# AnjieCheng/SpatialRGPT

Measured on AMD Instinct MI355X. Metric: region-grounded output tokens/sec @ VILA1.5-8B, 8 regions, greedy, higher is better.
Workload: dtype bf16; 1 GPU; BASELINE configs[1]: SpatialRGPT-VILA1.5-8B geometry (Llama-3-8B 32L/4096/GQA-8 + SigLIP-so400m 384px x2 passes + regiongpt extractor + mlp_downsample), 8 region masks, bs=1 per GPU, prompt 64 ids -> T=259, greedy 128 new tokens; parallelism=dp1, decode=hipGraph, llm_weights=bf16

## Files before the change

### spatialrgpt_amd/csrc/gemv.hip

```cpp
#include <stdlib.h>

#include <type_traits>

#include "common.h"
#include "gemv_route.h"
#include "internal.h"

namespace {

template <typename T>
struct WChunk;
template <>
struct WChunk<bf16_t> {
  static constexpr int VEC = 8;
  static __device__ __forceinline__ void cvt(const u32x4& r, float* f) {
#pragma unroll
    for (int i = 0; i < 4; ++i) {
      f[2 * i] = bf16lo(r[i]);
      f[2 * i + 1] = bf16hi(r[i]);
    }
  }
};
template <>
struct WChunk<float> {
  static constexpr int VEC = 4;
  static __device__ __forceinline__ void cvt(const u32x4& r, float* f) {
#pragma unroll
    for (int i = 0; i < 4; ++i) f[i] = __uint_as_float(r[i]);
  }
};

template <typename T, int B, bool SWIGLU, int NXMAX, int UB = 8>
__global__ __launch_bounds__(256, 2) void gemv_kernel(const T* __restrict__ x, const T* __restrict__ W,
                                                      const T* __restrict__ norm_w, float norm_eps,
                                                      const T* __restrict__ residual, void* __restrict__ out, int N,
                                                      int K, int out_f32) {
  constexpr int VEC = WChunk<T>::VEC;
  constexpr int R = SWIGLU ? 2 : 1;
  constexpr int U = UB / R;
  extern __shared__ __attribute__((aligned(16))) unsigned char smem[];
  T* xs = reinterpret_cast<T*>(smem);
  __shared__ float red[16];
  constexpr int RES_MAXU = 4;
  __shared__ float res_s[B][4][RES_MAXU];

  const int tid = threadIdx.x, lane = tid & 63, wave = tid >> 6;
  const int nchunks = K / VEC;
  const int nit = (nchunks + 63) >> 6;

  u32x4 w[R][U];
  auto issue = [&](int unit, int it0) {
#pragma unroll
    for (int r = 0; r < R; ++r) {
      const u32x4* p = reinterpret_cast<const u32x4*>(W + (size_t)(unit + r * N) * K);
#pragma unroll
      for (int j = 0; j < U; ++j) {
        w[r][j] = __builtin_nontemporal_load(p + min((it0 + j) * 64 + lane, nchunks - 1));
        __builtin_amdgcn_sched_barrier(0);
      }
    }
  };

  {
    const int total = B * nchunks;
    const bool do_norm = norm_w != nullptr;
    Vec16<T> xr[NXMAX], gr[NXMAX];
    const int rb = tid / (4 * RES_MAXU), rw = (tid / RES_MAXU) & 3, rk = tid % RES_MAXU;
    const int runit = (int)blockIdx.x * 4 + rw + rk * (int)gridDim.x * 4;
    const bool rok = !SWIGLU && residual != nullptr && tid < B * 4 * RES_MAXU && runit < N;
    const T res_raw = (residual != nullptr ? residual : x)[rok ? (size_t)rb * N + runit : 0];
#pragma unroll
    for (int j = 0; j < NXMAX; ++j) {
      const int c = (tid + 256 * j) % total;
      xr[j] = *reinterpret_cast<const Vec16<T>*>(x + (size_t)c * VEC);
      gr[j] = *reinterpret_cast<const Vec16<T>*>((do_norm ? norm_w : x) + (size_t)(c % nchunks) * VEC);
    }
    __builtin_amdgcn_sched_barrier(0);
    issue(min((int)blockIdx.x * 4 + wave, N - 1), 0);
    __builtin_amdgcn_sched_barrier(0);
    float ss[B];
#pragma unroll
    for (int b = 0; b < B; ++b) ss[b] = 0.f;
#pragma unroll
    for (int j = 0; j < NXMAX; ++j) {
      const int c = tid + 256 * j;
      const bool ok = c < total;
      float sq = 0.f;
#pragma unroll
      for (int i = 0; i < VEC; ++i) sq += xr[j].get(i) * xr[j].get(i);
      const int b = (B == 1) ? 0 : (c % total) / nchunks;
#pragma unroll
      for (int bb = 0; bb < B; ++bb) ss[bb] += (ok && bb == b) ? sq : 0.f;
    }
    for (int c = tid + 256 * NXMAX; c < total; c += 256) {
      const Vec16<T> v = *reinterpret_cast<const Vec16<T>*>(x + (size_t)c * VEC);
      *reinterpret_cast<Vec16<T>*>(xs + (size_t)c * VEC) = v;
      const int b = c / nchunks;
      float sq = 0.f;
#pragma unroll
      for (int i = 0; i < VEC; ++i) sq += v.get(i) * v.get(i);
#pragma unroll
      for (int bb = 0; bb < B; ++bb)
        if (bb == b) ss[bb] += sq;
    }
    if (rok) res_s[rb][rw][rk] = to_f(res_raw);
    float rs[B];
#pragma unroll
    for (int b = 0; b < B; ++b) rs[b] = 1.f;
    if (do_norm) {
#pragma unroll
      for (int b = 0; b < B; ++b) rs[b] = rsqrtf(block_sum(ss[b], red) / (float)K + norm_eps);
    }
#pragma unroll
    for (int j = 0; j < NXMAX; ++j) {
      const int c = tid + 256 * j;
      if (c < total) {
        Vec16<T> v = xr[j];
        if (do_norm) {
          const int b = (B == 1) ? 0 : c / nchunks;
          float r = rs[0];
#pragma unroll
          for (int bb = 1; bb < B; ++bb)
            if (bb == b) r = rs[bb];
#pragma unroll
          for (int i = 0; i < VEC; ++i) v.set(i, gr[j].get(i) * rnd<T>(xr[j].get(i) * r));
        }
        *reinterpret_cast<Vec16<T>*>(xs + (size_t)c * VEC) = v;
      }
    }
    if (do_norm) {
      for (int c = tid + 256 * NXMAX; c < total; c += 256) {
        const int b = c / nchunks, kc = c - b * nchunks;
        Vec16<T> v = *reinterpret_cast<Vec16<T>*>(xs + (size_t)c * VEC);
        const Vec16<T> g = *reinterpret_cast<const Vec16<T>*>(norm_w + (size_t)kc * VEC);
        float r = rs[0];
#pragma unroll
        for (int bb = 1; bb < B; ++bb)
          if (bb == b) r = rs[bb];
#pragma unroll
        for (int i = 0; i < VEC; ++i) v.set(i, g.get(i) * rnd<T>(v.get(i) * r));
        *reinterpret_cast<Vec16<T>*>(xs + (size_t)c * VEC) = v;
      }
    }
    __syncthreads();
  }

  int uk = 0;
  for (int unit = blockIdx.x * 4 + wave; unit < N; unit += gridDim.x * 4, ++uk) {
    float acc[R][B];
#pragma unroll
    for (int r = 0; r < R; ++r)
#pragma unroll
      for (int b = 0; b < B; ++b) acc[r][b] = 0.f;

    for (int it0 = 0; it0 < nit; it0 += U) {
#pragma unroll
      for (int j = 0; j < U; ++j) {
        const int ch = (it0 + j) * 64 + lane;
        const bool valid = ch < nchunks;
        const int chc = valid ? ch : nchunks - 1;
        float wf[R][VEC];
#pragma unroll
        for (int r = 0; r < R; ++r) {
          u32x4 wv = w[r][j];
#pragma unroll
          for (int q = 0; q < 4; ++q) wv[q] = valid ? wv[q] : 0u;
          WChunk<T>::cvt(wv, wf[r]);
        }
#pragma unroll
        for (int b = 0; b < B; ++b) {
          const Vec16<T> xv = *reinterpret_cast<const Vec16<T>*>(xs + (size_t)b * K + (size_t)chc * VEC);
#pragma unroll
          for (int i = 0; i < VEC; ++i) {
            const float xf = xv.get(i);
#pragma unroll
            for (int r = 0; r < R; ++r) acc[r][b] = fmaf(wf[r][i], xf, acc[r][b]);
          }
        }
      }
      {
        const bool more = it0 + U < nit;
        issue(more ? unit : min(unit + (int)gridDim.x * 4, N - 1), more ? it0 + U : 0);
      }
    }

#pragma unroll
    for (int b = 0; b < B; ++b) {
      float a[R];
#pragma unroll
      for (int r = 0; r < R; ++r) a[r] = wave_sum(acc[r][b]);
      if (lane == 0) {
        if (SWIGLU) {
          const float g = rnd<T>(a[0]), u = rnd<T>(a[R - 1]);
          reinterpret_cast<T*>(out)[(size_t)b * N + unit] = from_f<T>(rnd<T>(silu(g)) * u);
        } else {
          float v = rnd<T>(a[0]);
          if (residual) v = rnd<T>((uk < RES_MAXU ? res_s[b][wave][uk] : to_f(residual[(size_t)b * N + unit])) + v);
          if (out_f32)
            reinterpret_cast<float*>(out)[(size_t)b * N + unit] = v;
          else
            reinterpret_cast<T*>(out)[(size_t)b * N + unit] = from_f<T>(v);
        }
      }
    }
  }
}

template <bool SWIGLU, bool NORM, int NIT, int UB = 8>
__global__ __launch_bounds__(256, 2) void gemv_reg_kernel(const bf16_t* __restrict__ x, const bf16_t* __restrict__ W,
                                                          const bf16_t* __restrict__ norm_w, float norm_eps,
                                                          const bf16_t* __restrict__ residual, void* __restrict__ out, int N,
                                                          int K, int out_f32) {
  typedef bf16_t T;
  constexpr int VEC = 8;
  constexpr int R = SWIGLU ? 2 : 1;
  constexpr int U = UB / R;
  constexpr int RES_MAXU = 4;
  const int tid = threadIdx.x, lane = tid & 63, wave = tid >> 6;
  const int nchunks = K / VEC;

  u32x4 w[R][U];
  auto issue = [&](int unit, auto it0_c) {
    constexpr int IT0 = decltype(it0_c)::value;
#pragma unroll
    for (int r = 0; r < R; ++r) {
      const u32x4* p = reinterpret_cast<const u32x4*>(W + (size_t)(unit + r * N) * K);
#pragma unroll
      for (int j = 0; j < U; ++j) {
        if (IT0 + j < NIT) {
          w[r][j] = __builtin_nontemporal_load(p + min((IT0 + j) * 64 + lane, nchunks - 1));
          __builtin_amdgcn_sched_barrier(0);
        }
      }
    }
  };

  u32x4 xp[NIT];
  unsigned int res_raw;
// ... 65 lines not shown
        }
      }
    };
    batch(std::integral_constant<int, 0>{});
    if constexpr (U < NIT) batch(std::integral_constant<int, U>{});
    if constexpr (2 * U < NIT) batch(std::integral_constant<int, 2 * U>{});
    if constexpr (3 * U < NIT) batch(std::integral_constant<int, 3 * U>{});
    static_assert(4 * U >= NIT, "gemv_reg_kernel: at most 4 batches per row");
    float a[R];
#pragma unroll
    for (int r = 0; r < R; ++r) a[r] = wave_sum(acc[r]);
    const float res_b = __uint_as_float((unsigned int)__builtin_amdgcn_readlane((int)res_raw, uk < RES_MAXU ? uk : 0) << 16);
    if (lane == 0) {
      if (SWIGLU) {
        const float g = rnd<T>(a[0]), u = rnd<T>(a[R - 1]);
        reinterpret_cast<T*>(out)[unit] = from_f<T>(rnd<T>(silu(g)) * u);
      } else {
        float v = rnd<T>(a[0]);
        if (residual) v = rnd<T>((uk < RES_MAXU ? res_b : to_f(residual[unit])) + v);
        if (out_f32)
          reinterpret_cast<float*>(out)[unit] = v;
        else
          reinterpret_cast<T*>(out)[unit] = from_f<T>(v);
      }
    }
  }
}

template <typename T>
int launch_gemv(GemvFamily family, const DecodeProduct& p, hipStream_t s) {
  const GemvValuLaunch l = gemv_valu_launch(family, p.batch, p.N, p.K, sizeof(T) == 2, p.swiglu != 0, srgpt_device_cus());
  SRGPT_CHECK(l.lds <= GEMV_LDS_CAP, SRGPT_ERR_UNSUPPORTED, "srgpt_gemv: batch*K too large for LDS (%zu bytes)", (size_t)l.lds);
  const T *x = (const T*)p.x, *W = (const T*)p.W, *norm_w = (const T*)p.norm_w, *residual = (const T*)p.residual;
  SRGPT_TRY((srgpt_switch<false, true>(p.swiglu != 0, "SWIGLU", [&](auto sw_c) {
    constexpr bool SW = decltype(sw_c)::value;
    if constexpr (sizeof(T) == 2) {
      if (family == GEMV_REG)
        return srgpt_switch<5, 8, 14>(l.NIT, "NIT", [&](auto nit_c) {
          hipLaunchKernelGGL((gemv_reg_kernel<SW, false, decltype(nit_c)::value>), dim3(l.grid), dim3(256), 0, s, x, W, norm_w, p.eps,
                             residual, p.out, p.N, p.K, p.out_f32);
          return (int)SRGPT_OK;
        });
    }
    return srgpt_switch<1, 2, 3, 4>(l.B, "B", [&](auto b_c) {
      return srgpt_switch<2, 8>(l.NX, "NX", [&](auto nx_c) {
        constexpr int B = decltype(b_c)::value, NX = decltype(nx_c)::value;
        const auto go = [&](auto ub_c) {
          constexpr auto kfn = &gemv_kernel<T, B, SW, NX, decltype(ub_c)::value>;
          return srgpt_launch_dyn_lds<kfn>(l.raise_lds_limit ? GEMV_LDS_CAP : 0, dim3(l.grid), dim3(256), (size_t)l.lds, s, x, W, norm_w,
                                           p.eps, residual, p.out, p.N, p.K, p.out_f32);
        };
        if constexpr (!SW && NX == 8) {
          if (l.UB == 7) return go(std::integral_constant<int, 7>{});
        }
        return go(std::integral_constant<int, 8>{});
      });
    });
  })));
  SRGPT_LAUNCH_CHECK();
  return SRGPT_OK;
}

}

int srgpt_decode_product(const DecodeProduct& p, hipStream_t s) {
  const bool bf16 = p.dtype == SRGPT_BF16;
  const GemvRoute r = gemv_route(p.batch, p.K, bf16, p.fp8 != 0, p.norm_w != nullptr);
  const size_t es = dtype_size(p.dtype), on = p.out_f32 ? sizeof(float) : es;
  for (int b0 = 0; b0 < p.batch; b0 += r.chunk) {
    DecodeProduct c = p;
    c.batch = p.batch - b0 < r.chunk ? p.batch - b0 : r.chunk;
    c.x = (const char*)p.x + (size_t)b0 * p.K * es;
    if (p.residual) c.residual = (const char*)p.residual + (size_t)b0 * p.N * es;
    c.out = (char*)p.out + (size_t)b0 * p.N * on;
    if (p.ss_in) c.ss_in = p.ss_in + (size_t)b0 * SRGPT_ROWSS_STRIDE;
    if (p.ss_out) c.ss_out = p.ss_out + (size_t)b0 * SRGPT_ROWSS_STRIDE;
    switch (r.family) {
      case GEMV_SKINNY: SRGPT_TRY(srgpt_skinny_launch(c, s)); break;
      case GEMV_W8: SRGPT_TRY(srgpt_gemv_w8_valu(c, s)); break;
      default: SRGPT_TRY(bf16 ? launch_gemv<bf16_t>(r.family, c, s) : launch_gemv<float>(r.family, c, s));
    }
  }
  return SRGPT_OK;
}

extern "C" int srgpt_gemv(const void* x, const void* W, const void* norm_w, float norm_eps, const void* residual,
                          void* out, int batch, int N, int K, int swiglu, int out_f32, int dtype,
                          srgpt_stream_t stream) {
  SRGPT_CHECK(x && W && out, SRGPT_ERR_ARG, "srgpt_gemv: null pointer");
  SRGPT_CHECK(N > 0 && K > 0 && batch > 0, SRGPT_ERR_ARG, "srgpt_gemv: bad shape");
  SRGPT_CHECK(dtype == SRGPT_F32 || dtype == SRGPT_BF16, SRGPT_ERR_ARG, "srgpt_gemv: bad dtype %d", dtype);
  const int vec = dtype == SRGPT_BF16 ? 8 : 4;
  SRGPT_CHECK(K % vec == 0, SRGPT_ERR_ARG, "srgpt_gemv: K=%d must be a multiple of %d", K, vec);
  SRGPT_CHECK(!(swiglu && (residual || out_f32)), SRGPT_ERR_ARG, "srgpt_gemv: swiglu excludes residual/out_f32");
  return srgpt_decode_product(DecodeProduct{x, W, nullptr, norm_w, norm_eps, residual, out, batch, N, K, swiglu, out_f32, dtype, 0,
                                            nullptr, nullptr, 0},
                              as_stream(stream));
}

static_assert(GEMV_ROWSS_SLOTS == SRGPT_ROWSS_STRIDE, "gemv_route.h counts the slots of include/srgpt.h's tables");
extern "C" int srgpt_gemv_rowss_supported(int batch, int dtype, int fp8) {
// ... 21 lines not shown
```

### spatialrgpt_amd/csrc/internal.h

```cpp
#pragma once
#include "common.h"

struct SrgptGemmEpilogue;
struct GemmRoute;

int srgpt_gemm256_launch(const void* A, const void* W, int K, int lda, const SrgptGemmEpilogue& e, hipStream_t s);
int srgpt_gemm288_launch(const void* A, const void* W, int K, int lda, const SrgptGemmEpilogue& e, hipStream_t s);

void srgpt_splitk_apply(SrgptGemmEpilogue& e, const GemmRoute& r, void* ws);
int srgpt_splitk_finish(const SrgptGemmEpilogue& e, hipStream_t s, bool* fused);

struct DecodeProduct {
  const void *x, *W;
  const float* wscale;
  const void* norm_w;
  float eps;
  const void* residual;
  void* out;
  int batch, N, K, swiglu, out_f32, dtype, fp8;
  const float* ss_in;
  float* ss_out;
  int packed;
};
int srgpt_decode_product(const DecodeProduct& p, hipStream_t s);
int srgpt_skinny_launch(const DecodeProduct& p, hipStream_t s);
int srgpt_gemv_w8_valu(const DecodeProduct& p, hipStream_t s);

int srgpt_decode_attention_pf(const void* qkv, void* kcache, void* vcache, const int* pos, const void* cos_tab,
                              const void* sin_tab, void* out, float* ws, int B, int Hq, int Hkv, int D, int max_pos, int dtype,
                              const void* next_w, int next_n, int next_k, int next_fp8, srgpt_stream_t stream);
void* srgpt_decode_attn_sync_words(float* ws, int B, int Hq, int D, size_t* bytes);

int srgpt_sample_launch(const float* logits, const srgpt_sampling* sp, int64_t* tok, void* ws, float* pv, int* pi, int* err, int B, int V,
                        hipStream_t s);
int srgpt_sample_full_launch(const float* logits, const srgpt_sampling* sp, void* keys_thr, float* pv, int* pi, unsigned* kept_mask, int B,
                             int V, hipStream_t s);

int srgpt_logits_proc_launch(float* scores, const srgpt_logits_proc* lp, const int64_t* ids, int ld, int n, const int* n_dev, int B, int V,
                             hipStream_t s);
int srgpt_logits_proc_max_history();

struct AttnArgs {
  const bf16_t *q, *k, *v;
  bf16_t* o;
  int Tq, Tk, Hq, Hkv, D;
  int64_t q_bs, q_ts, q_hs, k_bs, k_ts, k_hs, v_bs, v_ts, v_hs;
  float scale;
  const int* kv_len;
};
int64_t srgpt_flash_slice_span_limit();
void srgpt_flash_bf16_launch(const AttnArgs& a, int B, bool causal, hipStream_t s);
```

### spatialrgpt_amd/csrc/model.hip

```cpp
#include <vector>

#include "common.h"
#include "gemv_route.h"
#include "internal.h"
#include "pick.h"

namespace {

inline size_t align256(size_t x) { return (x + 255) & ~(size_t)255; }

struct Carver {
  char* base;
  size_t off = 0;
  explicit Carver(void* p) : base(reinterpret_cast<char*>(p)) {}
  void* take(size_t bytes) {
    void* r = base ? base + off : nullptr;
    off += align256(bytes);
    return r;
  }
};

struct VitWs {
  void *col, *h, *qkv, *mlp, *gws;
  size_t gws_bytes, total;
};
VitWs carve_vit(const srgpt_vit_weights* w, int n_img, void* ws) {
  const size_t es = dtype_size(w->dtype);
  const int g = w->image_size / w->patch;
  const size_t rows = (size_t)n_img * (g * g + (w->cls_emb ? 1 : 0));
  Carver c(ws);
  VitWs v;
  v.col = c.take(rows * w->kp * es);
  v.h = c.take(rows * w->hidden * es);
  v.qkv = c.take(rows * 3 * w->hidden * es);
  v.mlp = c.take(rows * w->inter_pad * es);
  v.gws_bytes = (size_t)srgpt_gemm_ws_bytes((int)rows, w->hidden);
  v.gws = c.take(v.gws_bytes);
  v.total = c.off;
  return v;
}

struct LlmWs {
  void *x, *h, *qkv, *attn, *gu, *act, *last;
  void *xd, *qkvd, *attnd, *actd;
  float* dws;
  void* gws;
  size_t gws_bytes;
  float* amax_v;
  int* amax_i;
  int64_t* tok_emb;
  void* smp;
  void* smpf;
  int* err;
  float* rowss;
  void* a8;
  float* a8s;
  size_t total;
};
LlmWs carve_llm(const srgpt_llm_weights* w, int batch, int max_tokens, void* ws) {
  const size_t es = dtype_size(w->dtype);
  const size_t rows = (size_t)batch * max_tokens;
  const size_t qkvw = (size_t)(w->heads + 2 * w->kv_heads) * w->head_dim;
  Carver c(ws);
  LlmWs l;
  l.x = c.take(rows * w->hidden * es);
  l.h = c.take(rows * w->hidden * es);
  l.qkv = c.take(rows * qkvw * es);
  l.attn = c.take(rows * (size_t)w->heads * w->head_dim * es);
  l.gu = c.take(rows * 2 * (size_t)w->inter * es);
  l.act = c.take(rows * (size_t)w->inter * es);
  l.last = c.take((size_t)batch * w->hidden * es);
  l.xd = c.take((size_t)batch * w->hidden * es);
  l.qkvd = c.take((size_t)batch * qkvw * es);
  l.attnd = c.take((size_t)batch * w->heads * w->head_dim * es);
  l.actd = c.take((size_t)batch * w->inter * es);
  l.dws = reinterpret_cast<float*>(c.take((size_t)srgpt_decode_attn_ws_floats(batch, w->heads, w->head_dim) * 4));
  l.gws_bytes = (size_t)srgpt_gemm_ws_bytes((int)rows, (int)(qkvw > (size_t)w->hidden ? qkvw : (size_t)w->hidden));
  l.gws = c.take(l.gws_bytes);
  l.amax_v = reinterpret_cast<float*>(c.take((size_t)batch * PICK_SLICES * 4));
  l.amax_i = reinterpret_cast<int*>(c.take((size_t)batch * PICK_SLICES * 4));
  l.tok_emb = reinterpret_cast<int64_t*>(c.take((size_t)batch * 8));
  l.err = reinterpret_cast<int*>(c.take(sizeof(int)));
  l.smp = c.take((size_t)carve_sample_ws(nullptr, batch).bytes);
  l.smpf = c.take(carve_sample_full_ws(nullptr, batch, w->vocab).head_bytes);
  l.rowss = reinterpret_cast<float*>(c.take((size_t)2 * batch * SRGPT_ROWSS_STRIDE * sizeof(float)));
  l.a8 = nullptr;
  l.a8s = nullptr;
  if (w->fp8_act) {
    size_t kmax = (size_t)w->hidden;
    if ((size_t)w->inter > kmax) kmax = (size_t)w->inter;
    if ((size_t)w->heads * w->head_dim > kmax) kmax = (size_t)w->heads * w->head_dim;
    l.a8 = c.take(rows * kmax);
    l.a8s = reinterpret_cast<float*>(c.take(rows * 4));
  }
  l.total = c.off;
  return l;
}

__global__ void set_int_kernel(int* p, int n, int v) {
  const int i = blockIdx.x * blockDim.x + threadIdx.x;
  if (i < n) p[i] = v;
}

__global__ __launch_bounds__(256) void argmax_partial_kernel(const float* __restrict__ logits, float* __restrict__ pv,
                                                             int* __restrict__ pi, int V) {
  const PickSlice sl = pick_slice(V);
  const float* row = logits + (size_t)blockIdx.y * V;
  float best = -INFINITY;
  int bi = PICK_NONE;
  for (int i = sl.lo + threadIdx.x; i < sl.hi; i += 256) {
    const float v = row[i];
    if (v > best) {
      best = v;
      bi = i;
    }
  }
// ... 72 lines not shown
  const int b = blockIdx.x * blockDim.x + threadIdx.x;
  if (b < B) tok_emb[b] = tok[b];
}

static inline bool advance_embeds(const srgpt_llm_weights* w, const srgpt_llm_state* st) {
  return st->batch <= ADVANCE_MAXB && ((size_t)w->hidden * dtype_size(w->dtype)) % 16 == 0;
}

struct Pick {
  int sampler;
  const srgpt_logits_proc* lp;
};

static int greedy_pick(const srgpt_llm_weights* w, srgpt_llm_state* st, const LlmWs& d, int bump_pos, Pick p, hipStream_t s) {
  const int B = st->batch;
  const bool emb = advance_embeds(w, st);
  if (p.lp) SRGPT_TRY(srgpt_logits_proc_launch(st->logits, p.lp, st->out_ids, st->max_new, 0, st->step, B, w->vocab, s));
  if (st->sampling) {
    if (p.sampler == SRGPT_SAMPLER_FULL)
      SRGPT_TRY(srgpt_sample_full_launch(st->logits, st->sampling, d.smpf, d.amax_v, d.amax_i, nullptr, B, w->vocab, s));
    else
      SRGPT_TRY(srgpt_sample_launch(st->logits, st->sampling, st->tok, d.smp, d.amax_v, d.amax_i, d.err, B, w->vocab, s));
  } else {
    hipLaunchKernelGGL(argmax_partial_kernel, dim3(PICK_SLICES, B), dim3(256), 0, s, st->logits, d.amax_v, d.amax_i, w->vocab);
  }
  hipLaunchKernelGGL(advance_kernel, dim3(1), dim3(B > 4 ? 1024 : 256), 0, s, d.amax_v, d.amax_i, PICK_SLICES, st->tok, st->out_ids,
                     st->pos, st->step, B, st->max_new, bump_pos, emb ? reinterpret_cast<const unsigned char*>(w->embed) : nullptr,
                     reinterpret_cast<unsigned char*>(d.xd), (int)((size_t)w->hidden * dtype_size(w->dtype)), d.tok_emb, st->sampling,
                     p.sampler == SRGPT_SAMPLER_TOPK64 ? 1 : 0);
  SRGPT_LAUNCH_CHECK();
  return SRGPT_OK;
}

}

struct srgpt_graph {
  hipGraph_t graph;
  hipGraphExec_t exec;
};

extern "C" int64_t srgpt_vit_ws_bytes(const srgpt_vit_weights* w, int n_img) {
  if (!w || n_img <= 0) return -1;
  return (int64_t)carve_vit(w, n_img, nullptr).total;
}

extern "C" int srgpt_vit_forward(const srgpt_vit_weights* w, const void* images, void* out, void* ws, int n_img,
                                 srgpt_stream_t stream) {
  SRGPT_CHECK(w && images && out && ws && n_img > 0, SRGPT_ERR_ARG, "srgpt_vit_forward: bad args");
  SRGPT_CHECK(w->hidden % w->heads == 0 && w->image_size >= w->patch, SRGPT_ERR_ARG, "srgpt_vit_forward: bad config");
  SRGPT_CHECK(w->inter_pad >= w->inter && w->inter_pad % 8 == 0, SRGPT_ERR_ARG, "srgpt_vit_forward: inter_pad %d < inter %d",
              w->inter_pad, w->inter);
  const int dt = w->dtype, C = w->hidden, I = w->inter, IP = w->inter_pad, H = w->heads, hd = C / H;
  const int g = w->image_size / w->patch, gg = g * g, L = gg + (w->cls_emb ? 1 : 0), rows = n_img * L;
  const VitWs v = carve_vit(w, n_img, ws);
  void* x = out;
  SRGPT_TRY(srgpt_im2col(images, v.col, n_img, w->image_size, w->patch, w->kp, dt, stream));
  if (!w->cls_emb) {
    SRGPT_TRY(srgpt_gemm(v.col, w->patch_w, w->patch_b, w->pos_emb, x, rows, C, w->kp, w->kp, C, SRGPT_ACT_NONE, 0, L, 0,
                         SRGPT_OUT_PLAIN, 0, v.gws, (int64_t)v.gws_bytes, dt, stream));
  } else {
    SRGPT_TRY(srgpt_gemm(v.col, w->patch_w, w->patch_b, nullptr, v.h, n_img * gg, C, w->kp, w->kp, C, SRGPT_ACT_NONE, 0, 0, 0,
                         SRGPT_OUT_PLAIN, 0, v.gws, (int64_t)v.gws_bytes, dt, stream));
    SRGPT_TRY(srgpt_vit_assemble_cls(v.h, w->cls_emb, w->pos_emb, x, n_img, gg, C, dt, stream));
    if (w->pre_ln_w) SRGPT_TRY(srgpt_layernorm(x, w->pre_ln_w, w->pre_ln_b, x, rows, C, w->eps, SRGPT_ACT_NONE, dt, stream));
  }
  const float scale = 1.0f / sqrtf((float)hd);
  const char* qkv = reinterpret_cast<const char*>(v.qkv);
  const size_t es = dtype_size(dt);
  if (IP > I)
    SRGPT_HIP_TRY(hipMemset2DAsync(reinterpret_cast<char*>(v.mlp) + (size_t)I * es, (size_t)IP * es, 0, (size_t)(IP - I) * es,
                                   (size_t)rows, as_stream(stream)),
// ... 167 lines not shown
    SRGPT_TRY(gemm_w8a8(m.gu, nullptr, l.gu, 2 * I, Hd));
    SRGPT_TRY(srgpt_silu_mul(l.gu, l.act, rows, I, dt, stream));
    SRGPT_TRY(quant(l.act, I));
    return gemm_w8a8(m.down, l.x, l.x, Hd, I);
  }
};

}

static int prefill_impl(const srgpt_llm_weights* w, srgpt_llm_state* st, const void* inputs_embeds, int T, const int* lens,
                        float* all_logits, void* hidden_out, srgpt_stream_t stream) {
  SRGPT_TRY(check_llm(w, st));
  SRGPT_CHECK(inputs_embeds && T > 0 && T <= st->max_pos, SRGPT_ERR_ARG, "srgpt_llm_prefill: T=%d exceeds max_pos=%d", T,
              st->max_pos);
  SRGPT_CHECK(T <= st->ws_tokens, SRGPT_ERR_ARG, "srgpt_llm_prefill: T=%d exceeds ws_tokens=%d", T, st->ws_tokens);
  LlmFormat fmt;
  SRGPT_TRY(llm_format(w, "srgpt_llm_prefill", &fmt));
  const int dt = w->dtype, Hd = w->hidden, I = w->inter, Hq = w->heads, D = w->head_dim;
  const int B = st->batch, rows = B * T;
  if (fmt == FMT_W8A8)
    SRGPT_CHECK(Hd % 128 == 0 && I % 128 == 0 && (Hq * D) % 128 == 0 && Hd >= 256 && I >= 256 && Hq * D >= 256,
                SRGPT_ERR_UNSUPPORTED, "srgpt_llm_prefill: fp8_act needs hidden, inter and heads * head_dim to be multiples of 128");
  const bool wide = Hd > 16384 || I > 16384;
  const size_t es = dtype_size(dt);
  hipStream_t s = as_stream(stream);
  const Prefill p{w, st, carve_llm(w, B, st->ws_tokens, st->ws), fmt, B, T, rows, Hd, I, Hq * D, (Hq + 2 * w->kv_heads) * D, dt, stream};
  const LlmWs& l = p.l;
  const size_t hid_bytes = (size_t)rows * Hd * es;
  {
    size_t sync_bytes = 0;
    void* sync = srgpt_decode_attn_sync_words(l.dws, B, Hq, D, &sync_bytes);
    SRGPT_HIP_TRY(hipMemsetAsync(sync, 0, sync_bytes, s), "srgpt_llm_prefill: re-arming the decode tickets");
    SRGPT_HIP_TRY(hipMemsetAsync(l.tok_emb, 0xFF, (size_t)B * sizeof(int64_t), s), "srgpt_llm_prefill: resetting the embedded-token record");
    SRGPT_HIP_TRY(hipMemsetAsync(l.err, 0, sizeof(int), s), "srgpt_llm_prefill: clearing the decode error word");
  }
  if (hipMemcpyAsync(l.x, inputs_embeds, hid_bytes, hipMemcpyDeviceToDevice, s) != hipSuccess) {
    srgpt_set_error("srgpt_llm_prefill: memcpy failed");
    return SRGPT_ERR_LAUNCH;
  }
  if (hidden_out) SRGPT_HIP_TRY(hipMemcpyAsync(hidden_out, l.x, hid_bytes, hipMemcpyDeviceToDevice, s), "srgpt_llm_prefill: hidden-state copy");
  for (int i = 0; i < w->layers; ++i) {
    switch (fmt) {
      case FMT_DTYPE: SRGPT_TRY(p.layer_dtype(i)); break;
      case FMT_W8A16: SRGPT_TRY(p.layer_w8a16(i)); break;
      case FMT_W8A8: SRGPT_TRY(wide ? p.layer_w8a8_wide(i) : p.layer_w8a8(i)); break;
    }
    if (hidden_out)
      SRGPT_HIP_TRY(hipMemcpyAsync(reinterpret_cast<char*>(hidden_out) + (size_t)(i + 1) * hid_bytes, l.x, hid_bytes,
                                   hipMemcpyDeviceToDevice, s),
                    "srgpt_llm_prefill: hidden-state copy");
  }
  if (all_logits) {
    SRGPT_TRY(p.norm(w->final_norm));
    if (fmt == FMT_DTYPE)
      SRGPT_TRY(srgpt_gemm(l.h, w->lm_head, nullptr, nullptr, all_logits, rows, w->vocab, Hd, Hd, w->vocab, SRGPT_ACT_NONE, 0, 0, 1,
                           SRGPT_OUT_PLAIN, 0, nullptr, 0, dt, stream));
    else
      SRGPT_TRY(srgpt_gemm_w8(l.h, w->lm_head8, w->lm_head_scale, nullptr, nullptr, all_logits, rows, w->vocab, Hd, Hd, w->vocab,
                              SRGPT_ACT_NONE, 1, nullptr, 0, stream));
  }
  if (lens) {
    SRGPT_CHECK(Hd % (16 / (int)es) == 0, SRGPT_ERR_ARG, "srgpt_llm_prefill_ragged: hidden %d not a multiple of 16 bytes", Hd);
    if (dt == SRGPT_BF16)
      hipLaunchKernelGGL(gather_last_rows_kernel<bf16_t>, dim3(B), dim3(256), 0, s, (const bf16_t*)l.x, lens, (bf16_t*)l.last,
                         st->pos, T, Hd);
    else
      hipLaunchKernelGGL(gather_last_rows_kernel<float>, dim3(B), dim3(256), 0, s, (const float*)l.x, lens, (float*)l.last,
// ... 61 lines not shown
namespace {

struct DecodeStep {
  const srgpt_llm_weights* w;
  int B;
  bool fp8, pub;
  srgpt_stream_t stream;

  int gemv(const Mat& m, const void* x, const void* norm, const void* res, void* out, int N, int K, int swiglu, int f32,
           const float* ss_in, float* ss_out) const {
    if (pub)
      return srgpt_gemv_rowss(x, m.w, m.pk ? m.pk : m.w8, m.scale, norm, w->rms_eps, res, out, B, N, K, swiglu, f32, ss_in, ss_out,
                              m.pk ? m.pk_rows : 0, stream);
    if (fp8) return srgpt_gemv_w8(x, m.w8, m.scale, norm, w->rms_eps, res, out, B, N, K, swiglu, f32, stream);
    return srgpt_gemv(x, m.w, norm, w->rms_eps, res, out, B, N, K, swiglu, f32, w->dtype, stream);
  }
};

}

static int decode_step_impl(const srgpt_llm_weights* w, srgpt_llm_state* st, srgpt_stream_t stream, bool embed_first, Pick p) {
  LlmFormat fmt;
  SRGPT_TRY(llm_format(w, "srgpt_llm_decode_step", &fmt));
  const int dt = w->dtype, Hd = w->hidden, I = w->inter, Hq = w->heads, Hkv = w->kv_heads, D = w->head_dim;
  const int B = st->batch, QW = (Hq + 2 * Hkv) * D;
  const size_t es = dtype_size(dt);
  hipStream_t s = as_stream(stream);
  const LlmWs d = carve_llm(w, B, st->ws_tokens, st->ws);
  const size_t layer_kv = (size_t)B * Hkv * st->max_pos * D * es;
  if (embed_first) {
    SRGPT_TRY(srgpt_embed_rows(w->embed, st->tok, d.xd, B, Hd, dt, stream));
    hipLaunchKernelGGL(record_embedded_kernel, dim3(cdiv(B, 64)), dim3(64), 0, s, st->tok, d.tok_emb, B);
    SRGPT_LAUNCH_CHECK();
  } else {
    hipLaunchKernelGGL(embed_sync_kernel, dim3(B < 64 ? B : 64), dim3(256), 0, s, st->tok, d.tok_emb,
                       reinterpret_cast<const unsigned char*>(w->embed), reinterpret_cast<unsigned char*>(d.xd), B, (int)((size_t)Hd * es),
                       (int64_t)w->vocab, d.err);
    SRGPT_LAUNCH_CHECK();
  }
  const bool fp8 = fmt != FMT_DTYPE;
  const DecodeStep ds{w, B, fp8, gemv_rowss_supported(B, dt == SRGPT_BF16, fp8, srgpt_device_cus()), stream};
  float* const ss_attn = d.rowss;
  float* const ss_mlp = d.rowss + (size_t)B * SRGPT_ROWSS_STRIDE;
  for (int i = 0; i < w->layers; ++i) {
    char* kc = reinterpret_cast<char*>(st->kcache) + (size_t)i * layer_kv;
    char* vc = reinterpret_cast<char*>(st->vcache) + (size_t)i * layer_kv;
    const LayerMats m = layer_mats(w, fmt, i);
    SRGPT_TRY(ds.gemv(m.qkv, d.xd, w->attn_norm[i], nullptr, d.qkvd, QW, Hd, 0, 0, i > 0 ? ss_mlp : nullptr, nullptr));
    SRGPT_TRY(srgpt_decode_attention_pf(d.qkvd, kc, vc, st->pos, w->rope_cos, w->rope_sin, d.attnd, d.dws, B, Hq, Hkv, D,
                                        st->max_pos, dt, fp8 ? m.o.w8 : m.o.w, Hd, Hq * D, fp8 ? 1 : 0, stream));
    SRGPT_TRY(ds.gemv(m.o, d.attnd, nullptr, d.xd, d.xd, Hd, Hq * D, 0, 0, nullptr, ss_attn));
    SRGPT_TRY(ds.gemv(m.gu, d.xd, w->mlp_norm[i], nullptr, d.actd, I, Hd, 1, 0, ss_attn, nullptr));
    SRGPT_TRY(ds.gemv(m.down, d.actd, nullptr, d.xd, d.xd, Hd, I, 0, 0, nullptr, ss_mlp));
  }
  SRGPT_TRY(ds.gemv(Mat{w->lm_head, w->lm_head8, w->lm_head_scale, nullptr, 0}, d.xd, w->final_norm, nullptr, st->logits, w->vocab, Hd,
                    0, 1, w->layers > 0 ? ss_mlp : nullptr, nullptr));
  return greedy_pick(w, st, d, 1, p, s);
}

extern "C" int srgpt_llm_decode_step_ex(const srgpt_llm_weights* w, srgpt_llm_state* st, int sampler, srgpt_stream_t stream) {
  SRGPT_TRY(check_pick(w, st, Pick{sampler, nullptr}, "srgpt_llm_decode_step_ex"));
  return decode_step_impl(w, st, stream, true, Pick{sampler, nullptr});
}

extern "C" int srgpt_llm_decode_step_proc(const srgpt_llm_weights* w, srgpt_llm_state* st, int sampler, const srgpt_logits_proc* lp,
                                          srgpt_stream_t stream) {
  SRGPT_TRY(check_pick(w, st, Pick{sampler, lp}, "srgpt_llm_decode_step_proc"));
  return decode_step_impl(w, st, stream, true, Pick{sampler, lp});
}

extern "C" int srgpt_llm_decode_step(const srgpt_llm_weights* w, srgpt_llm_state* st, srgpt_stream_t stream) {
  SRGPT_TRY(check_pick(w, st, Pick{SRGPT_SAMPLER_TOPK64, nullptr}, "srgpt_llm_decode_step"));
  return decode_step_impl(w, st, stream, true, Pick{SRGPT_SAMPLER_TOPK64, nullptr});
}

extern "C" int srgpt_llm_decode_sync_state(const srgpt_llm_weights* w, const srgpt_llm_state* st, srgpt_stream_t stream) {
  SRGPT_TRY(check_llm(w, st));
  const LlmWs d = carve_llm(w, st->batch, st->ws_tokens, st->ws);
  size_t bytes = 0;
  void* sync = srgpt_decode_attn_sync_words(d.dws, st->batch, w->heads, w->head_dim, &bytes);
  std::vector<int> host(bytes / sizeof(int) + 1);
  SRGPT_HIP_TRY(hipMemcpyAsync(host.data(), sync, bytes, hipMemcpyDeviceToHost, as_stream(stream)), "srgpt_llm_decode_sync_state: copy");
  SRGPT_HIP_TRY(hipMemcpyAsync(&host.back(), d.err, sizeof(int), hipMemcpyDeviceToHost, as_stream(stream)), "srgpt_llm_decode_sync_state: copy");
  SRGPT_HIP_TRY(hipStreamSynchronize(as_stream(stream)), "srgpt_llm_decode_sync_state: synchronize");
  const size_t n = host.size() - 1;
  for (size_t i = 0; i < n; ++i)
    SRGPT_CHECK(host[i] == 0, SRGPT_ERR_STATE, "decode step: arrival ticket %zu of %zu is %d between steps (expected 0)", i, n, host[i]);
  SRGPT_CHECK((host.back() & 4) == 0, SRGPT_ERR_UNSUPPORTED,
              "decode step: sampling parameters the device sampler does not serve (top_k > 64, or top_p < 1 without top_k): the draws "
              "used another distribution");
  SRGPT_CHECK((host.back() & 2) == 0, SRGPT_ERR_STATE,
              "decode step: more than 256 vocabulary entries tie at the top-k threshold of a sampling step (kept set truncated)");
  SRGPT_CHECK((host.back() & 1) == 0, SRGPT_ERR_STATE,
              "decode step: a token id written into st->tok lies outside the embedding table [0, %d); the step ran on a stale row",
              w->vocab);
  return SRGPT_OK;
}

static int check_graph(const srgpt_llm_weights* w, const srgpt_llm_state* st, Pick p, srgpt_graph** out, const char* fn) {
  SRGPT_CHECK(out, SRGPT_ERR_ARG, "srgpt_llm_decode_graph_create: null out");
  return check_pick(w, st, p, fn);
}

static int graph_create_impl(const srgpt_llm_weights* w, srgpt_llm_state* st, Pick p, srgpt_stream_t stream, srgpt_graph** out) {
  LlmFormat fmt;
  SRGPT_TRY(llm_format(w, "srgpt_llm_decode_step", &fmt));
  hipStream_t s = as_stream(stream);
  (void)srgpt_device_cus();
  hipGraph_t graph = nullptr;
  if (hipStreamBeginCapture(s, hipStreamCaptureModeThreadLocal) != hipSuccess) {
    srgpt_set_error("hipStreamBeginCapture failed");
    return SRGPT_ERR_STATE;
  }
  const int rc = decode_step_impl(w, st, stream, !advance_embeds(w, st), p);
  const hipError_t ee = hipStreamEndCapture(s, &graph);
  if (rc != SRGPT_OK) {
    if (graph) (void)hipGraphDestroy(graph);
    return rc;
  }
  if (ee != hipSuccess || !graph) {
    srgpt_set_error("hipStreamEndCapture failed: %s", hipGetErrorString(ee));
    return SRGPT_ERR_STATE;
  }
  hipGraphExec_t exec = nullptr;
  const hipError_t ei = hipGraphInstantiate(&exec, graph, nullptr, nullptr, 0);
  if (ei != hipSuccess) {
    (void)hipGraphDestroy(graph);
    srgpt_set_error("hipGraphInstantiate failed: %s", hipGetErrorString(ei));
    return SRGPT_ERR_STATE;
  }
  *out = new srgpt_graph{graph, exec};
  return SRGPT_OK;
}

extern "C" int srgpt_llm_decode_graph_create_ex(const srgpt_llm_weights* w, srgpt_llm_state* st, int sampler, srgpt_stream_t stream,
                                                srgpt_graph** out) {
  SRGPT_TRY(check_graph(w, st, Pick{sampler, nullptr}, out, "srgpt_llm_decode_graph_create_ex"));
  return graph_create_impl(w, st, Pick{sampler, nullptr}, stream, out);
}

extern "C" int srgpt_llm_decode_graph_create_proc(const srgpt_llm_weights* w, srgpt_llm_state* st, int sampler,
                                                  const srgpt_logits_proc* lp, srgpt_stream_t stream, srgpt_graph** out) {
  SRGPT_TRY(check_graph(w, st, Pick{sampler, lp}, out, "srgpt_llm_decode_graph_create_proc"));
  return graph_create_impl(w, st, Pick{sampler, lp}, stream, out);
}

extern "C" int srgpt_llm_decode_graph_create(const srgpt_llm_weights* w, srgpt_llm_state* st, srgpt_stream_t stream,
                                             srgpt_graph** out) {
  SRGPT_TRY(check_graph(w, st, Pick{SRGPT_SAMPLER_TOPK64, nullptr}, out, "srgpt_llm_decode_graph_create"));
  return graph_create_impl(w, st, Pick{SRGPT_SAMPLER_TOPK64, nullptr}, stream, out);
}

extern "C" int srgpt_graph_launch(srgpt_graph* g, int times, srgpt_stream_t stream) {
  SRGPT_CHECK(g && times >= 0, SRGPT_ERR_ARG, "srgpt_graph_launch: bad args");
  for (int i = 0; i < times; ++i) {
    const hipError_t e = hipGraphLaunch(g->exec, as_stream(stream));
    if (e != hipSuccess) {
      srgpt_set_error("hipGraphLaunch failed: %s", hipGetErrorString(e));
      return SRGPT_ERR_LAUNCH;
    }
  }
  return SRGPT_OK;
}

extern "C" int srgpt_graph_destroy(srgpt_graph* g) {
  if (!g) return SRGPT_OK;
  (void)hipGraphExecDestroy(g->exec);
  (void)hipGraphDestroy(g->graph);
  delete g;
  return SRGPT_OK;
}
```

### spatialrgpt_amd/csrc/pick.h

```cpp
#pragma once
#include "common.h"

constexpr int PICK_SLICES = 128;
constexpr int PICK_SLICE_MAX = 2048;
constexpr int PICK_VOCAB_MAX = PICK_SLICES * PICK_SLICE_MAX;
constexpr int PICK_NONE = 0x7fffffff;
constexpr int SMP_K = 64;

static inline int pick_check_vocab(int V, const char* who) {
  SRGPT_CHECK(V <= PICK_VOCAB_MAX, SRGPT_ERR_UNSUPPORTED, "%s: vocabulary %d exceeds %d", who, V, PICK_VOCAB_MAX);
  return SRGPT_OK;
}

struct SampleWs {
  unsigned* cand_key;
  int* cand_idx;
  float* pv;
  int* pi;
  int* err;
  int64_t bytes;
};
static inline SampleWs carve_sample_ws(const void* ws, int B) {
  const uintptr_t p = reinterpret_cast<uintptr_t>(ws), cand = (uintptr_t)B * PICK_SLICES * SMP_K * 4, part = (uintptr_t)B * PICK_SLICES * 4;
  return SampleWs{reinterpret_cast<unsigned*>(p), reinterpret_cast<int*>(p + cand), reinterpret_cast<float*>(p + 2 * cand),
                  reinterpret_cast<int*>(p + 2 * cand + part), reinterpret_cast<int*>(p + 2 * cand + 2 * part),
                  (int64_t)(2 * cand + 2 * part + 256)};
}
struct SampleFullWs {
  unsigned *keys, *thr;
  float* pv;
  int* pi;
  size_t head_bytes;
  int64_t bytes;
};
static inline SampleFullWs carve_sample_full_ws(const void* ws, int B, int V) {
  const uintptr_t p = reinterpret_cast<uintptr_t>(ws), keys = (uintptr_t)B * V * 4, head = keys + (uintptr_t)B * 16;
  const uintptr_t part = (uintptr_t)B * PICK_SLICES * 4;
  return SampleFullWs{reinterpret_cast<unsigned*>(p), reinterpret_cast<unsigned*>(p + keys), reinterpret_cast<float*>(p + head),
                      reinterpret_cast<int*>(p + head + part), (size_t)head, (int64_t)(head + 2 * part)};
}

__device__ __forceinline__ bool pick_better(float v, int i, float ov, int oi) { return v > ov || (v == ov && i < oi); }

struct PickSlice {
  int lo, hi;
};
__device__ __forceinline__ PickSlice pick_slice(int V) {
  const int per = (V + gridDim.x - 1) / gridDim.x, lo = blockIdx.x * per;
  return PickSlice{lo, min(lo + per, V)};
}

__device__ __forceinline__ void pick_wave_reduce(float& v, int& i) {
#pragma unroll
  for (int o = 32; o > 0; o >>= 1) {
    const float ov = __shfl_xor(v, o);
    const int oi = __shfl_xor(i, o);
    if (pick_better(ov, oi, v, i)) {
      v = ov;
      i = oi;
    }
  }
}

__device__ __forceinline__ void pick_store_slice(float v, int i, float* __restrict__ pv, int* __restrict__ pi) {
  __shared__ float sv[4];
  __shared__ int si[4];
  pick_wave_reduce(v, i);
  if ((threadIdx.x & 63) == 0) {
    sv[threadIdx.x >> 6] = v;
    si[threadIdx.x >> 6] = i;
  }
  __syncthreads();
  if (threadIdx.x == 0) {
    for (int w = 1; w < 4; ++w)
      if (pick_better(sv[w], si[w], v, i)) {
// ... 40 lines not shown
```

Baseline: 335.2 tokens/s.

## Fuse greedy argmax and next-token embedding into the lm_head GEMV tail

The lm_head GEMV tracks a per-wave running argmax. The last-arriving block, found through an atomic ticket, merges the per-block partials, writes the token and output id, bumps pos and step, and copies the next token's embedding row into the decode input. This removes the separate greedy-pick kernels and the per-step embed-sync kernel from the decode graph. The embed sync now runs once before graph launches. In exchange it adds a grid-wide ticket, a serialized tail in one block, and a NORM template switch that skips norm-weight loads when there is no norm.

Measured after the change: 334.8 tokens/s. Within noise of the previous version (-0.1%).

```diff
diff --git a/spatialrgpt_amd/csrc/gemv.hip b/spatialrgpt_amd/csrc/gemv.hip
--- a/spatialrgpt_amd/csrc/gemv.hip
+++ b/spatialrgpt_amd/csrc/gemv.hip
@@ -5,6 +5,7 @@
 #include "common.h"
 #include "gemv_route.h"
 #include "internal.h"
+#include "pick.h"
 
 namespace {
 
@@ -30,11 +31,86 @@
   }
 };
 
-template <typename T, int B, bool SWIGLU, int NXMAX, int UB = 8>
+__device__ __forceinline__ void gemv_pick_tail(float pick_v, int pick_i, int tid, int lane, int wave, const PickTail& pk) {
+  __shared__ float pk_v[4];
+  __shared__ int pk_i[4], pk_last, pk_tok;
+  if (lane == 0) {
+    pk_v[wave] = pick_v;
+    pk_i[wave] = pick_i;
+  }
+  __syncthreads();
+  if (tid == 0) {
+    float v = pk_v[0];
+    int i = pk_i[0];
+    for (int w = 1; w < 4; ++w)
+      if (pick_better(pk_v[w], pk_i[w], v, i)) {
+        v = pk_v[w];
+        i = pk_i[w];
+      }
+    __hip_atomic_store(pk.partials + blockIdx.x, pick_pack(v, i), __ATOMIC_RELAXED, __HIP_MEMORY_SCOPE_AGENT);
+    asm volatile("s_waitcnt vmcnt(0)" ::: "memory");
+    const int t = __hip_atomic_fetch_add(pk.ticket, 1, __ATOMIC_ACQ_REL, __HIP_MEMORY_SCOPE_AGENT);
+    pk_last = t == (int)gridDim.x - 1;
+  }
+  __syncthreads();
+  if (!pk_last) return;
+  const int s = *pk.step;
+  if (wave == 0) {
+    const int nb = (int)gridDim.x;
+    float best = -INFINITY;
+    int bi = PICK_NONE;
+    for (int i0 = 0; i0 < nb; i0 += 8 * 64) {
+      unsigned long long u[8];
+#pragma unroll
+      for (int j = 0; j < 8; ++j)
+        u[j] = __hip_atomic_load(pk.partials + min(i0 + j * 64 + lane, nb - 1), __ATOMIC_RELAXED, __HIP_MEMORY_SCOPE_AGENT);
+#pragma unroll
+      for (int j = 0; j < 8; ++j) {
+        const float v = pick_unpack_v(u[j]);
+        const int i = pick_unpack_i(u[j]);
+        if (i0 + j * 64 + lane < nb && pick_better(v, i, best, bi)) {
+          best = v;
+          bi = i;
+        }
+      }
+    }
+    pick_wave_reduce(best, bi);
+    if (lane == 0) {
+      const int64_t t = bi == PICK_NONE ? 0 : bi;
+      pk.tok[0] = t;
+      if (pk.embed) {
+        pk_tok = (int)t;
+        pk.tok_emb[0] = t;
+      }
+      if (s < pk.max_new) pk.out_ids[s] = t;
+      if (pk.bump_pos) pk.pos[0] += 1;
+    }
+  }
+  __syncthreads();
+  if (tid == 0) *pk.step = s + 1;
+  if (pk.embed) {
+    const int total = pk.row_bytes >> 4;
+    const unsigned char* src = pk.embed + (size_t)pk_tok * pk.row_bytes;
+    for (int i0 = tid; i0 < total; i0 += 4 * 256) {
+      u32x4 v[4];
+#pragma unroll
+      for (int u = 0; u < 4; ++u) v[u] = *reinterpret_cast<const u32x4*>(src + (size_t)min(i0 + u * 256, total - 1) * 16);
+#pragma unroll
+      for (int u = 0; u < 4; ++u)
+        if (i0 + u * 256 < total) *reinterpret_cast<u32x4*>(pk.xd + (size_t)(i0 + u * 256) * 16) = v[u];
+    }
+  }
+  if (tid == 0) __hip_atomic_store(pk.ticket, 0, __ATOMIC_RELAXED, __HIP_MEMORY_SCOPE_AGENT);
+}
+
+template <typename T, int B, bool SWIGLU, int NXMAX, int UB = 8, bool NORM = true, typename... PICKARG>
 __global__ __launch_bounds__(256, 2) void gemv_kernel(const T* __restrict__ x, const T* __restrict__ W,
                                                       const T* __restrict__ norm_w, float norm_eps,
                                                       const T* __restrict__ residual, void* __restrict__ out, int N,
-                                                      int K, int out_f32) {
+                                                      int K, int out_f32, PICKARG... pick) {
+  constexpr bool PICK = sizeof...(PICKARG) == 1;
+  static_assert(sizeof...(PICKARG) <= 1 && (std::is_same_v<PICKARG, PickTail> && ...), "gemv_kernel: at most one PickTail");
+  static_assert(!PICK || (B == 1 && !SWIGLU && sizeof(T) == 2), "gemv_kernel: the pick rides on one bf16 row of plain products");
   constexpr int VEC = WChunk<T>::VEC;
   constexpr int R = SWIGLU ? 2 : 1;
   constexpr int U = UB / R;
@@ -63,8 +139,8 @@
 
   {
     const int total = B * nchunks;
-    const bool do_norm = norm_w != nullptr;
-    Vec16<T> xr[NXMAX], gr[NXMAX];
+    const bool do_norm = NORM && norm_w != nullptr;
+    Vec16<T> xr[NXMAX], gr[NORM ? NXMAX : 1];
     const int rb = tid / (4 * RES_MAXU), rw = (tid / RES_MAXU) & 3, rk = tid % RES_MAXU;
     const int runit = (int)blockIdx.x * 4 + rw + rk * (int)gridDim.x * 4;
     const bool rok = !SWIGLU && residual != nullptr && tid < B * 4 * RES_MAXU && runit < N;
@@ -73,7 +149,7 @@
     for (int j = 0; j < NXMAX; ++j) {
       const int c = (tid + 256 * j) % total;
       xr[j] = *reinterpret_cast<const Vec16<T>*>(x + (size_t)c * VEC);
-      gr[j] = *reinterpret_cast<const Vec16<T>*>((do_norm ? norm_w : x) + (size_t)(c % nchunks) * VEC);
+      if constexpr (NORM) gr[j] = *reinterpret_cast<const Vec16<T>*>((do_norm ? norm_w : x) + (size_t)(c % nchunks) * VEC);
     }
     __builtin_amdgcn_sched_barrier(0);
     issue(min((int)blockIdx.x * 4 + wave, N - 1), 0);
@@ -123,7 +199,7 @@
           for (int bb = 1; bb < B; ++bb)
             if (bb == b) r = rs[bb];
 #pragma unroll
-          for (int i = 0; i < VEC; ++i) v.set(i, gr[j].get(i) * rnd<T>(xr[j].get(i) * r));
+          for (int i = 0; i < VEC; ++i) v.set(i, gr[NORM ? j : 0].get(i) * rnd<T>(xr[j].get(i) * r));
         }
         *reinterpret_cast<Vec16<T>*>(xs + (size_t)c * VEC) = v;
       }
@@ -145,6 +221,8 @@
     __syncthreads();
   }
 
+  float pick_v = -INFINITY;
+  int pick_i = PICK_NONE;
   int uk = 0;
   for (int unit = blockIdx.x * 4 + wave; unit < N; unit += gridDim.x * 4, ++uk) {
     float acc[R][B];
@@ -200,10 +278,18 @@
             reinterpret_cast<float*>(out)[(size_t)b * N + unit] = v;
           else
             reinterpret_cast<T*>(out)[(size_t)b * N + unit] = from_f<T>(v);
-        }
-      }
-    }
-  }
+          if constexpr (PICK) {
+            if (v > pick_v) {
+              pick_v = v;
+              pick_i = unit;
+            }
+          }
+        }
+      }
+    }
+  }
+
+  if constexpr (PICK) gemv_pick_tail(pick_v, pick_i, tid, lane, wave, pick...);
 }
 
 template <bool SWIGLU, bool NORM, int NIT, int UB = 8>
@@ -335,6 +421,21 @@
   const GemvValuLaunch l = gemv_valu_launch(family, p.batch, p.N, p.K, sizeof(T) == 2, p.swiglu != 0, srgpt_device_cus());
   SRGPT_CHECK(l.lds <= GEMV_LDS_CAP, SRGPT_ERR_UNSUPPORTED, "srgpt_gemv: batch*K too large for LDS (%zu bytes)", (size_t)l.lds);
   const T *x = (const T*)p.x, *W = (const T*)p.W, *norm_w = (const T*)p.norm_w, *residual = (const T*)p.residual;
+  if (p.pick) {
+    if constexpr (sizeof(T) == 2) {
+      SRGPT_CHECK(family == GEMV_LDS && l.B == 1 && l.UB == 8 && norm_w && !residual && !p.swiglu && p.out_f32 &&
+                      l.grid <= PICK_TAIL_PARTIALS,
+                  SRGPT_ERR_UNSUPPORTED, "decode product: no kernel with the pick in its tail for this product");
+      SRGPT_TRY((srgpt_switch<2, 8>(l.NX, "NX", [&](auto nx_c) {
+        constexpr auto kfn = &gemv_kernel<T, 1, false, decltype(nx_c)::value, 8, true, PickTail>;
+        return srgpt_launch_dyn_lds<kfn>(l.raise_lds_limit ? GEMV_LDS_CAP : 0, dim3(l.grid), dim3(256), (size_t)l.lds, s, x, W, norm_w,
+                                         p.eps, residual, p.out, p.N, p.K, p.out_f32, *p.pick);
+      })));
+      SRGPT_LAUNCH_CHECK();
+      return SRGPT_OK;
+    }
+    SRGPT_CHECK(false, SRGPT_ERR_UNSUPPORTED, "decode product: the pick in the tail needs bf16");
+  }
   SRGPT_TRY((srgpt_switch<false, true>(p.swiglu != 0, "SWIGLU", [&](auto sw_c) {
     constexpr bool SW = decltype(sw_c)::value;
     if constexpr (sizeof(T) == 2) {
@@ -349,9 +450,11 @@
       return srgpt_switch<2, 8>(l.NX, "NX", [&](auto nx_c) {
         constexpr int B = decltype(b_c)::value, NX = decltype(nx_c)::value;
         const auto go = [&](auto ub_c) {
-          constexpr auto kfn = &gemv_kernel<T, B, SW, NX, decltype(ub_c)::value>;
-          return srgpt_launch_dyn_lds<kfn>(l.raise_lds_limit ? GEMV_LDS_CAP : 0, dim3(l.grid), dim3(256), (size_t)l.lds, s, x, W, norm_w,
-                                           p.eps, residual, p.out, p.N, p.K, p.out_f32);
+          return srgpt_switch<false, true>(norm_w != nullptr, "NORM", [&](auto norm_c) {
+            constexpr auto kfn = &gemv_kernel<T, B, SW, NX, decltype(ub_c)::value, decltype(norm_c)::value>;
+            return srgpt_launch_dyn_lds<kfn>(l.raise_lds_limit ? GEMV_LDS_CAP : 0, dim3(l.grid), dim3(256), (size_t)l.lds, s, x, W,
+                                             norm_w, p.eps, residual, p.out, p.N, p.K, p.out_f32);
+          });
         };
         if constexpr (!SW && NX == 8) {
           if (l.UB == 7) return go(std::integral_constant<int, 7>{});
@@ -370,6 +473,8 @@
   const bool bf16 = p.dtype == SRGPT_BF16;
   const GemvRoute r = gemv_route(p.batch, p.K, bf16, p.fp8 != 0, p.norm_w != nullptr);
   const size_t es = dtype_size(p.dtype), on = p.out_f32 ? sizeof(float) : es;
+  SRGPT_CHECK(!p.pick || (r.family == GEMV_LDS && p.batch == 1), SRGPT_ERR_UNSUPPORTED,
+              "decode product: the pick in the tail is served for one row on the LDS kernel");
   for (int b0 = 0; b0 < p.batch; b0 += r.chunk) {
     DecodeProduct c = p;
     c.batch = p.batch - b0 < r.chunk ? p.batch - b0 : r.chunk;
diff --git a/spatialrgpt_amd/csrc/internal.h b/spatialrgpt_amd/csrc/internal.h
--- a/spatialrgpt_amd/csrc/internal.h
+++ b/spatialrgpt_amd/csrc/internal.h
@@ -10,6 +10,18 @@
 void srgpt_splitk_apply(SrgptGemmEpilogue& e, const GemmRoute& r, void* ws);
 int srgpt_splitk_finish(const SrgptGemmEpilogue& e, hipStream_t s, bool* fused);
 
+constexpr int PICK_TAIL_PARTIALS = 1024;
+struct PickTail {
+  unsigned long long* partials;
+  int* ticket;
+  int64_t *tok, *out_ids;
+  int *pos, *step;
+  int max_new, bump_pos;
+  const unsigned char* embed;
+  unsigned char* xd;
+  int row_bytes;
+  int64_t* tok_emb;
+};
 struct DecodeProduct {
   const void *x, *W;
   const float* wscale;
@@ -21,6 +33,7 @@
   const float* ss_in;
   float* ss_out;
   int packed;
+  const PickTail* pick = nullptr;
 };
 int srgpt_decode_product(const DecodeProduct& p, hipStream_t s);
 int srgpt_skinny_launch(const DecodeProduct& p, hipStream_t s);
diff --git a/spatialrgpt_amd/csrc/model.hip b/spatialrgpt_amd/csrc/model.hip
--- a/spatialrgpt_amd/csrc/model.hip
+++ b/spatialrgpt_amd/csrc/model.hip
@@ -48,6 +48,8 @@
   size_t gws_bytes;
   float* amax_v;
   int* amax_i;
+  unsigned long long* pick_pairs;
+  int* pick_ticket;
   int64_t* tok_emb;
   void* smp;
   void* smpf;
@@ -81,7 +83,10 @@
   l.amax_i = reinterpret_cast<int*>(c.take((size_t)batch * PICK_SLICES * 4));
   l.tok_emb = reinterpret_cast<int64_t*>(c.take((size_t)batch * 8));
   l.err = reinterpret_cast<int*>(c.take(sizeof(int)));
+  l.pick_ticket = l.err ? l.err + 4 : nullptr;
   l.smp = c.take((size_t)carve_sample_ws(nullptr, batch).bytes);
+  static_assert((size_t)PICK_TAIL_PARTIALS * 8 <= (size_t)PICK_SLICES * SMP_K * 4, "the pairs fit one row's candidate keys");
+  l.pick_pairs = reinterpret_cast<unsigned long long*>(l.smp);
   l.smpf = c.take(carve_sample_full_ws(nullptr, batch, w->vocab).head_bytes);
   l.rowss = reinterpret_cast<float*>(c.take((size_t)2 * batch * SRGPT_ROWSS_STRIDE * sizeof(float)));
   l.a8 = nullptr;
@@ -220,11 +225,29 @@
   return SRGPT_OK;
 }
 
-}
-
+static bool pick_in_tail(const srgpt_llm_weights* w, const srgpt_llm_state* st, bool fp8, Pick p) {
+  if (st->sampling || p.lp || st->batch != 1 || fp8 || w->dtype != SRGPT_BF16) return false;
+  if (!w->lm_head || !w->final_norm || w->vocab <= 0 || w->hidden <= 0 || w->hidden % 8 != 0) return false;
+  if (gemv_route(1, w->hidden, true, false, true).family != GEMV_LDS) return false;
+  const GemvValuLaunch l = gemv_valu_launch(GEMV_LDS, 1, w->vocab, w->hidden, true, false, srgpt_device_cus());
+  return l.UB == 8 && l.grid <= PICK_TAIL_PARTIALS;
+}
+
+}
+
+struct GraphEmbedSync {
+  const int64_t* tok;
+  int64_t* tok_emb;
+  const unsigned char* embed;
+  unsigned char* xd;
+  int B, row_bytes;
+  int64_t vocab;
+  int* err;
+};
 struct srgpt_graph {
   hipGraph_t graph;
   hipGraphExec_t exec;
+  GraphEmbedSync sync;
 };
 
 extern "C" int64_t srgpt_vit_ws_bytes(const srgpt_vit_weights* w, int n_img) {
@@ -458,7 +481,7 @@
     void* sync = srgpt_decode_attn_sync_words(l.dws, B, Hq, D, &sync_bytes);
     SRGPT_HIP_TRY(hipMemsetAsync(sync, 0, sync_bytes, s), "srgpt_llm_prefill: re-arming the decode tickets");
     SRGPT_HIP_TRY(hipMemsetAsync(l.tok_emb, 0xFF, (size_t)B * sizeof(int64_t), s), "srgpt_llm_prefill: resetting the embedded-token record");
-    SRGPT_HIP_TRY(hipMemsetAsync(l.err, 0, sizeof(int), s), "srgpt_llm_prefill: clearing the decode error word");
+    SRGPT_HIP_TRY(hipMemsetAsync(l.err, 0, 32, s), "srgpt_llm_prefill: clearing the decode error word and the pick's ticket");
   }
   if (hipMemcpyAsync(l.x, inputs_embeds, hid_bytes, hipMemcpyDeviceToDevice, s) != hipSuccess) {
     srgpt_set_error("srgpt_llm_prefill: memcpy failed");
@@ -586,11 +609,6 @@
     SRGPT_TRY(srgpt_embed_rows(w->embed, st->tok, d.xd, B, Hd, dt, stream));
     hipLaunchKernelGGL(record_embedded_kernel, dim3(cdiv(B, 64)), dim3(64), 0, s, st->tok, d.tok_emb, B);
     SRGPT_LAUNCH_CHECK();
-  } else {
-    hipLaunchKernelGGL(embed_sync_kernel, dim3(B < 64 ? B : 64), dim3(256), 0, s, st->tok, d.tok_emb,
-                       reinterpret_cast<const unsigned char*>(w->embed), reinterpret_cast<unsigned char*>(d.xd), B, (int)((size_t)Hd * es),
-                       (int64_t)w->vocab, d.err);
-    SRGPT_LAUNCH_CHECK();
   }
   const bool fp8 = fmt != FMT_DTYPE;
   const DecodeStep ds{w, B, fp8, gemv_rowss_supported(B, dt == SRGPT_BF16, fp8, srgpt_device_cus()), stream};
@@ -607,6 +625,15 @@
     SRGPT_TRY(ds.gemv(m.gu, d.xd, w->mlp_norm[i], nullptr, d.actd, I, Hd, 1, 0, ss_attn, nullptr));
     SRGPT_TRY(ds.gemv(m.down, d.actd, nullptr, d.xd, d.xd, Hd, I, 0, 0, nullptr, ss_mlp));
   }
+  if (pick_in_tail(w, st, fp8, p)) {
+    const bool emb = advance_embeds(w, st);
+    const PickTail pt{d.pick_pairs, d.pick_ticket, st->tok, st->out_ids, st->pos, st->step, st->max_new, 1,
+                      emb ? reinterpret_cast<const unsigned char*>(w->embed) : nullptr, reinterpret_cast<unsigned char*>(d.xd),
+                      (int)((size_t)Hd * es), d.tok_emb};
+    return srgpt_decode_product(DecodeProduct{d.xd, w->lm_head, nullptr, w->final_norm, w->rms_eps, nullptr, st->logits, 1, w->vocab, Hd,
+                                              0, 1, dt, 0, nullptr, nullptr, 0, &pt},
+                                s);
+  }
   SRGPT_TRY(ds.gemv(Mat{w->lm_head, w->lm_head8, w->lm_head_scale, nullptr, 0}, d.xd, w->final_norm, nullptr, st->logits, w->vocab, Hd,
                     0, 1, w->layers > 0 ? ss_mlp : nullptr, nullptr));
   return greedy_pick(w, st, d, 1, p, s);
@@ -633,13 +660,15 @@
   const LlmWs d = carve_llm(w, st->batch, st->ws_tokens, st->ws);
   size_t bytes = 0;
   void* sync = srgpt_decode_attn_sync_words(d.dws, st->batch, w->heads, w->head_dim, &bytes);
-  std::vector<int> host(bytes / sizeof(int) + 1);
+  std::vector<int> host(bytes / sizeof(int) + 2);
+  const size_t n = host.size() - 2;
   SRGPT_HIP_TRY(hipMemcpyAsync(host.data(), sync, bytes, hipMemcpyDeviceToHost, as_stream(stream)), "srgpt_llm_decode_sync_state: copy");
+  SRGPT_HIP_TRY(hipMemcpyAsync(&host[n], d.pick_ticket, sizeof(int), hipMemcpyDeviceToHost, as_stream(stream)), "srgpt_llm_decode_sync_state: copy");
   SRGPT_HIP_TRY(hipMemcpyAsync(&host.back(), d.err, sizeof(int), hipMemcpyDeviceToHost, as_stream(stream)), "srgpt_llm_decode_sync_state: copy");
   SRGPT_HIP_TRY(hipStreamSynchronize(as_stream(stream)), "srgpt_llm_decode_sync_state: synchronize");
-  const size_t n = host.size() - 1;
   for (size_t i = 0; i < n; ++i)
     SRGPT_CHECK(host[i] == 0, SRGPT_ERR_STATE, "decode step: arrival ticket %zu of %zu is %d between steps (expected 0)", i, n, host[i]);
+  SRGPT_CHECK(host[n] == 0, SRGPT_ERR_STATE, "decode step: the pick's arrival ticket is %d between steps (expected 0)", host[n]);
   SRGPT_CHECK((host.back() & 4) == 0, SRGPT_ERR_UNSUPPORTED,
               "decode step: sampling parameters the device sampler does not serve (top_k > 64, or top_p < 1 without top_k): the draws "
               "used another distribution");
@@ -683,7 +712,13 @@
     srgpt_set_error("hipGraphInstantiate failed: %s", hipGetErrorString(ei));
     return SRGPT_ERR_STATE;
   }
-  *out = new srgpt_graph{graph, exec};
+  GraphEmbedSync sync{};
+  if (advance_embeds(w, st)) {
+    const LlmWs d = carve_llm(w, st->batch, st->ws_tokens, st->ws);
+    sync = GraphEmbedSync{st->tok, d.tok_emb, reinterpret_cast<const unsigned char*>(w->embed), reinterpret_cast<unsigned char*>(d.xd),
+                          st->batch, (int)((size_t)w->hidden * dtype_size(w->dtype)), (int64_t)w->vocab, d.err};
+  }
+  *out = new srgpt_graph{graph, exec, sync};
   return SRGPT_OK;
 }
 
@@ -707,6 +742,12 @@
 
 extern "C" int srgpt_graph_launch(srgpt_graph* g, int times, srgpt_stream_t stream) {
   SRGPT_CHECK(g && times >= 0, SRGPT_ERR_ARG, "srgpt_graph_launch: bad args");
+  if (times > 0 && g->sync.embed) {
+    const GraphEmbedSync& y = g->sync;
+    hipLaunchKernelGGL(embed_sync_kernel, dim3(y.B < 64 ? y.B : 64), dim3(256), 0, as_stream(stream), y.tok, y.tok_emb, y.embed, y.xd, y.B,
+                       y.row_bytes, y.vocab, y.err);
+    SRGPT_LAUNCH_CHECK();
+  }
   for (int i = 0; i < times; ++i) {
     const hipError_t e = hipGraphLaunch(g->exec, as_stream(stream));
     if (e != hipSuccess) {
diff --git a/spatialrgpt_amd/csrc/pick.h b/spatialrgpt_amd/csrc/pick.h
--- a/spatialrgpt_amd/csrc/pick.h
+++ b/spatialrgpt_amd/csrc/pick.h
@@ -41,6 +41,12 @@
 }
 
 __device__ __forceinline__ bool pick_better(float v, int i, float ov, int oi) { return v > ov || (v == ov && i < oi); }
+
+__device__ __forceinline__ unsigned long long pick_pack(float v, int i) {
+  return (unsigned long long)__float_as_uint(v) | ((unsigned long long)(unsigned)i << 32);
+}
+__device__ __forceinline__ float pick_unpack_v(unsigned long long u) { return __uint_as_float((unsigned)u); }
+__device__ __forceinline__ int pick_unpack_i(unsigned long long u) { return (int)(unsigned)(u >> 32); }
 
 struct PickSlice {
   int lo, hi;
```
